# poja/Cattus

Measured on AMD Instinct MI355X. Metric: MCTS node-evals/sec (chess 20x256 net, batch 256), higher is better.
Workload: dtype f16x2

## Files before the change

cattus_amd/csrc/evaluator.hip:

```cpp
#include <hip/hip_runtime.h>

#include <algorithm>
#include <atomic>
#include <chrono>
#include <condition_variable>
#include <cmath>
#include <cstdarg>
#include <cstdio>
#include <cstdlib>
#include <cstring>
#include <deque>
#include <functional>
#include <map>
#include <memory>
#include <mutex>
#include <new>
#include <shared_mutex>
#include <string>
#include <thread>
#include <vector>

#include <dlfcn.h>

#include "../../include/cattus_hip.h"
// ... 49 lines not shown
    return f;
}

std::vector<int> choose_stream_shift(const cattus_net_desc& d, const float* p, int* t) {
    const uint32_t F = d.filters;
    const float* g0 = p + (size_t)F * d.planes * 9;
    const float* b0 = g0 + F;
    const size_t stem = (size_t)F * d.planes * 9 + 4 * F, block = (size_t)2 * F * F * 9 + 6 * F;
    std::vector<double> s(F);
    for (uint32_t c = 0; c < F; c++) s[c] = (double)g0[c] * g0[c] + (double)b0[c] * b0[c];
    for (uint32_t i = 0; i < d.blocks; i++) {
        const float* g2 = p + stem + i * block + (size_t)F * F * 9 + 2 * F + (size_t)F * F * 9;
        const float* b2 = g2 + F;
        for (uint32_t c = 0; c < F; c++) s[c] += (double)g2[c] * g2[c] + (double)b2[c] * b2[c];
    }
    *t = stream_shift_global(s);
    return stream_shifts(s);
}

void shift_folded(Folded& f, uint32_t cin, const std::vector<int>& tk, bool writes) {
    const size_t cout = f.b.size();
    for (size_t i = 0; i < f.w.size(); i++) f.w[i] = ldexpf(f.w[i], writes ? tk[i / cin % cout] : -tk[i % cin]);
    for (size_t co = 0; writes && co < cout; co++) f.b[co] = ldexpf(f.b[co], tk[co]);
}

struct DevArena {
    char* base = nullptr;
    size_t cap = 0, used = 0;
    ~DevArena() {
        if (base) (void)hipFree(base);
    }
    void* take(size_t bytes) {
        const size_t at = (used + 4095) & ~(size_t)4095;
        if (!base || at + bytes > cap) return nullptr;
        used = at + bytes;
        return base + at;
    }
};

struct DevBuf {
    void* p = nullptr;
    bool owned = true;
    ~DevBuf() {
        if (p && owned) (void)hipFree(p);
    }
    int alloc(size_t bytes, DevArena* arena = nullptr) {
        if (p && owned) (void)hipFree(p);
        p = nullptr, owned = true;
        if (arena && (p = arena->take(bytes ? bytes : 16))) {
            owned = false;
            return CATTUS_OK;
        }
        hipError_t e = hipMalloc(&p, bytes ? bytes : 16);
        if (e != hipSuccess) return fail(CATTUS_E_NOMEM, "hipMalloc(%zu) failed: %s", bytes, hipGetErrorString(e));
        return CATTUS_OK;
    }
    int upload(const void* src, size_t bytes, DevArena* arena = nullptr) {
        int rc = alloc(bytes, arena);
        if (rc) return rc;
        HIP_TRY(hipMemcpy(p, src, bytes, hipMemcpyHostToDevice));
        return CATTUS_OK;
    }
    template <typename T>
    T* as() const {
        return reinterpret_cast<T*>(p);
    }
};

struct PinnedBuf {
    void* p = nullptr;
    ~PinnedBuf() {
        if (p) (void)hipHostFree(p);
    }
    int alloc(size_t bytes) {
        hipError_t e = hipHostMalloc(&p, bytes ? bytes : 16, hipHostMallocDefault);
        if (e != hipSuccess) return fail(CATTUS_E_NOMEM, "hipHostMalloc(%zu) failed: %s", bytes, hipGetErrorString(e));
        return CATTUS_OK;
    }
    template <typename T>
    T* as() const {
        return reinterpret_cast<T*>(p);
    }
};

std::shared_mutex g_pin_mu;
std::map<const char*, size_t> g_pinned;
struct Roctx {
    int (*push)(const char*) = nullptr;
    int (*pop)() = nullptr;
    Roctx() {
        const char* on = getenv("CATTUS_ROCTX");
        if (!on || on[0] != '1') return;
        for (const char* name : {"librocprofiler-sdk-roctx.so", "libroctx64.so"}) {
            if (void* h = dlopen(name, RTLD_NOW | RTLD_GLOBAL)) {
                push = reinterpret_cast<int (*)(const char*)>(dlsym(h, "roctxRangePushA"));
                pop = reinterpret_cast<int (*)()>(dlsym(h, "roctxRangePop"));
                if (push && pop) return;
                push = nullptr, pop = nullptr;
            }
        }
    }
};
const Roctx& roctx() {
    static const Roctx r;
    return r;
}
struct RoctxRange {
    bool on;
    RoctxRange(const char* what, uint32_t n) : on(roctx().push != nullptr) {
        if (on) {
            char buf[64];
            snprintf(buf, sizeof buf, "%s n=%u", what, n);
            roctx().push(buf);
        }
    }
    ~RoctxRange() {
        if (on) roctx().pop();
    }
};

bool is_pinned(const void* p) {
    std::shared_lock<std::shared_mutex> lk(g_pin_mu);
    auto it = g_pinned.upper_bound((const char*)p);
    if (it == g_pinned.begin()) return false;
    --it;
    return (const char*)p < it->first + it->second;
}

struct ConvLayer { DevBuf w, b; };

struct ServerBatch {
    uint64_t seq = 0;
    uint32_t count = 0, collected = 0;
    bool sealed = false, running = false, done = false;
    int status = CATTUS_OK;
    std::string error;
    std::chrono::steady_clock::time_point t0;
    std::vector<uint64_t> planes;
    std::vector<float> policy, value;
    std::vector<uint8_t> taken;
};

constexpr int NLANES = CATTUS_HIP_LANES;

struct Lane {
    hipStream_t stream = nullptr;
    hipEvent_t done = nullptr;
    DevBuf d_planes, x0, a, t, y, hv, h1, d_policy, d_value;
    DevBuf d_legal_idx, d_legal_cnt, d_probs;
    uint32_t legal_stride = 0;
    PinnedBuf h_planes, h_policy, h_value;
    DevBuf tower_layers, tower_ready;
    PinnedBuf h_tower_err;
    std::mutex mu;
    ~Lane() {
        if (done) (void)hipEventDestroy(done);
        if (stream) (void)hipStreamDestroy(stream);
    }
};

enum class TowerKind {
    Simple,
    Generic,
    PerLayer,
    Resident64,
    Resident64Split,
    Wino16,
    Wino4,
};
struct TowerPlan {
    TowerKind kind = TowerKind::Generic;
    bool w_frag = false;
    bool inplace = false;
    bool one_launch = false;
    bool tuned() const { return kind != TowerKind::Simple && kind != TowerKind::Generic; }
    bool wino() const { return kind == TowerKind::Wino16 || kind == TowerKind::Wino4; }
};

}

struct cattus_eval {
    DevArena arena;
    cattus_net_desc d{};
    cattus_eval_config cfg{};
    TowerPlan plan;
    DevBuf d1w, d1b, d2w, d2b, svw, svb, spw, spb;
    bool wait_spin = true;
    Act act = Act::F32;
    uint32_t hw = 0, bpad = 0, cpad0 = 0;
    uint32_t slots = 64;
    uint32_t fpad = 0;
    DevBuf t64_layers, t64s_bias;
    bool t64s_fuse_heads = true;
    int t64s_depth = 0;
    bool pack_separately = false;
    int t64_force_ch = 0;
    std::atomic<bool> tower_gave_up{false};
    uint32_t persist_spin = 1u << 18, cus = 0;
    bool stream_shift_on = true;
    int stream_shift = 0;
    std::vector<int> stream_shifts;
    ConvOpts conv_opts;
    DevBuf d_saturated;
    bool t64_layer_steps = true;
    int device = 0;

    ConvLayer stem;
    std::vector<std::unique_ptr<ConvLayer>> c1, c2;
    DevBuf head_w, head_b, w1t, b1, w2, b2, wpt, bp;
    uint32_t kvp = 0, kpp = 0;

    Lane lanes[NLANES];
    std::atomic<unsigned> lane_rr{0};

    std::mutex stat_mu;
    cattus_stats stats{};
    uint64_t stats_tower_fallbacks = 0;

    std::mutex srv_mu;
    std::condition_variable srv_cv, done_cv;
    std::deque<std::unique_ptr<ServerBatch>> batches;
    uint64_t next_seq = 1;
    bool flush_req = false, stop = false;
    std::thread servers[NLANES];

    ~cattus_eval() {
        {
            std::lock_guard<std::mutex> lk(srv_mu);
            stop = true;
        }
        srv_cv.notify_all();
        done_cv.notify_all();
        for (auto& t : servers)
            if (t.joinable()) t.join();
    }
};

namespace {

size_t blob_floats(const cattus_net_desc& d) {
    const size_t hw = (size_t)d.board * d.board, F = d.filters;
    if (F == 0) {
        const size_t K = (size_t)d.planes * hw;
        return 2 * (K * K + K) + K + 1 + (size_t)d.moves * K + d.moves;
    }
    size_t n = F * d.planes * 9 + 4 * F;
    n += (size_t)d.blocks * (2 * F * F * 9 + 6 * F);
    n += (size_t)d.vhc * F + 2 * (size_t)d.vhc + (size_t)FC_HIDDEN * d.vhc * hw + FC_HIDDEN + FC_HIDDEN + 1;
    n += (size_t)d.phc * F + 2 * (size_t)d.phc + (size_t)d.moves * d.phc * hw + d.moves;
    return n;
}

std::mutex g_chain_mu;
hipEvent_t g_chain[64] = {};
int chain_persistent_launch(int device, hipStream_t st, const std::function<void()>& launch) {
    std::lock_guard<std::mutex> lk(g_chain_mu);
    hipEvent_t& ev = g_chain[device & 63];
    if (!ev) {
        HIP_TRY(hipEventCreateWithFlags(&ev, hipEventDisableTiming));
    } else {
        HIP_TRY(hipStreamWaitEvent(st, ev, 0));
    }
    launch();
    HIP_TRY(hipEventRecord(ev, st));
    return CATTUS_OK;
}

int upload_conv(cattus_eval* e, ConvLayer& L, const Folded& f, uint32_t cout, uint32_t cin, bool stem = false) {
    auto up = [](DevBuf& buf, const auto& v, DevArena* arena = nullptr) { return buf.upload(v.data(), v.size() * sizeof(v[0]), arena); };
    int rc;
    if (!e->plan.tuned()) return (rc = up(L.b, f.b)) ? rc : up(L.w, f.w);
    const ConvShape s{cout, cin, e->fpad, stem ? e->cpad0 : e->fpad};
    if (e->plan.wino() && !stem) {
        std::vector<int> sh;
        const std::vector<double> U = wino_transform(f, s, &sh);
        if ((rc = up(L.b, bias_and_scales(f, s, &sh)))) return rc;
        return up(L.w, wino_u(U, s, sh), &e->arena);
    }
    const bool scaled = act_f16_family(e->act);
    const std::vector<int> sh = scaled ? channel_shifts(f, s) : std::vector<int>();
    if ((rc = up(L.b, bias_and_scales(f, s, scaled ? &sh : nullptr)))) return rc;
    if (e->act == Act::F32) return up(L.w, rows_f32(f, s));
    if (e->act == Act::BF16) return up(L.w, rows_bf16(f, s));
    if (e->act == Act::F16) return up(L.w, rows_f16(f, s, sh));
    return e->plan.w_frag ? up(L.w, frag_f16x2(f, s, sh)) : up(L.w, rows_f16x2(f, s, sh));
}

int lane_common(cattus_eval* e, Lane& L) {
    const size_t B = e->cfg.max_batch, M = e->d.moves, plane_bytes = B * e->d.planes * e->cfg.plane_words * 8;
    int rc;
    HIP_TRY(hipStreamCreateWithFlags(&L.stream, hipStreamNonBlocking));
    HIP_TRY(hipEventCreateWithFlags(&L.done, hipEventBlockingSync | hipEventDisableTiming));
    if ((rc = L.d_planes.alloc(plane_bytes)) || (rc = L.d_policy.alloc(B * M * 4)) || (rc = L.d_value.alloc(B * 4))) return rc;
    if ((rc = L.h_planes.alloc(plane_bytes)) || (rc = L.h_policy.alloc(B * M * 4)) || (rc = L.h_value.alloc(B * 4))) return rc;
    return CATTUS_OK;
}

uint32_t hv_leaves(const cattus_eval* e) { return (e->bpad + 31) / 32 * 32; }

int build_simple(cattus_eval* e, const float* p) {
    const cattus_net_desc& d = e->d;
    const size_t K = (size_t)d.planes * e->hw, M = d.moves, B = e->cfg.max_batch;
    auto upload_t = [&](DevBuf& buf, const float* w, size_t n_out) -> int {
        std::vector<float> t(K * n_out);
        for (size_t n = 0; n < n_out; n++)
            for (size_t k = 0; k < K; k++) t[k * n_out + n] = w[n * K + k];
        return buf.upload(t.data(), t.size() * 4);
    };
    int rc;
    const float *w1 = p, *b1 = w1 + K * K, *w2 = b1 + K, *b2 = w2 + K * K, *vw = b2 + K, *vb = vw + K, *pw = vb + 1, *pb = pw + M * K;
    if ((rc = upload_t(e->d1w, w1, K)) || (rc = e->d1b.upload(b1, K * 4)) || (rc = upload_t(e->d2w, w2, K)) || (rc = e->d2b.upload(b2, K * 4)) ||
        (rc = upload_t(e->svw, vw, 1)) || (rc = e->svb.upload(vb, 4)) || (rc = upload_t(e->spw, pw, M)) || (rc = e->spb.upload(pb, M * 4)))
        return rc;
    for (Lane& L : e->lanes)
        if ((rc = lane_common(e, L)) || (rc = L.x0.alloc(B * K * 4)) || (rc = L.a.alloc(B * K * 4)) || (rc = L.t.alloc(B * K * 4))) return rc;
    return CATTUS_OK;
}

int build(cattus_eval* e, const float* p) {
    const cattus_net_desc& d = e->d;
    const TowerPlan& plan = e->plan;
    if (plan.kind == TowerKind::Simple) return build_simple(e, p);
    const uint32_t F = d.filters, hw = e->hw, FP = e->fpad;
    auto take = [&](size_t n) { return (p += n) - n; };
    int rc;
    e->stream_shifts.assign(F, 0);
    if (act_f16_family(e->act) && e->stream_shift_on) e->stream_shifts = choose_stream_shift(d, p, &e->stream_shift);
    const std::vector<int>& tk = e->stream_shifts;
    const bool shifted = std::any_of(tk.begin(), tk.end(), [](int t) { return t != 0; });
    {
        const float* w = take((size_t)F * d.planes * 9);
        const float *g = take(F), *be = take(F), *mu = take(F), *var = take(F);
        Folded f = fold_conv(w, F, d.planes, 9, g, be, mu, var);
        if (shifted) shift_folded(f, d.planes, tk, true);
        if ((rc = upload_conv(e, e->stem, f, F, d.planes, true))) return rc;
    }
    for (uint32_t i = 0; i < d.blocks; i++) {
        e->c1.emplace_back(new ConvLayer);
        e->c2.emplace_back(new ConvLayer);
        const float* w1 = take((size_t)F * F * 9);
        const float *mu1 = take(F), *var1 = take(F);
        Folded f1 = fold_conv(w1, F, F, 9, nullptr, nullptr, mu1, var1);
        if (shifted) shift_folded(f1, F, tk, false);
        if ((rc = upload_conv(e, *e->c1.back(), f1, F, F))) return rc;
        const float* w2 = take((size_t)F * F * 9);
        const float *g2 = take(F), *be2 = take(F), *mu2 = take(F), *var2 = take(F);
        Folded f2 = fold_conv(w2, F, F, 9, g2, be2, mu2, var2);
        if (shifted) shift_folded(f2, F, tk, true);
        if ((rc = upload_conv(e, *e->c2.back(), f2, F, F))) return rc;
    }
    std::vector<float> hw_w((size_t)(d.vhc + d.phc) * F), hw_b(std::max(32u, d.vhc + d.phc), 0.0f);
    const float* vw = take((size_t)d.vhc * F);
    const float *vmu = take(d.vhc), *vvar = take(d.vhc);
    Folded fv = fold_conv(vw, d.vhc, F, 1, nullptr, nullptr, vmu, vvar);
    const float* fc1_w = take((size_t)FC_HIDDEN * d.vhc * hw);
    const float* fc1_b = take(FC_HIDDEN);
    const float* fc2_w = take(FC_HIDDEN);
    const float* fc2_b = take(1);
    const float* pw = take((size_t)d.phc * F);
    const float *pmu = take(d.phc), *pvar = take(d.phc);
    Folded fp = fold_conv(pw, d.phc, F, 1, nullptr, nullptr, pmu, pvar);
    const float* pfc_w = take((size_t)d.moves * d.phc * hw);
    const float* pfc_b = take(d.moves);
    if (shifted) shift_folded(fv, F, tk, false), shift_folded(fp, F, tk, false);
    memcpy(hw_w.data(), fv.w.data(), fv.w.size() * 4);
    memcpy(hw_w.data() + fv.w.size(), fp.w.data(), fp.w.size() * 4);
    memcpy(hw_b.data(), fv.b.data(), fv.b.size() * 4);
    memcpy(hw_b.data() + fv.b.size(), fp.b.data(), fp.b.size() * 4);
    const uint32_t kv = d.vhc * hw, kp = d.phc * hw;
    if ((rc = e->head_b.upload(hw_b.data(), hw_b.size() * 4)) || (rc = e->b1.upload(fc1_b, FC_HIDDEN * 4)) || (rc = e->w2.upload(fc2_w, FC_HIDDEN * 4)) ||
        (rc = e->b2.upload(fc2_b, 4)) || (rc = e->bp.upload(pfc_b, d.moves * 4)))
        return rc;
    if (plan.tuned()) {
        const uint32_t ocn = d.vhc + d.phc;
        e->kvp = (kv + 15) / 16 * 16;
        e->kpp = (kp + 15) / 16 * 16;
        const uint32_t m32 = (d.moves + 31) / 32 * 32;
        std::vector<float> cw((size_t)32 * FP, 0.0f), w1((size_t)FC_HIDDEN * e->kvp, 0.0f), wp((size_t)m32 * e->kpp, 0.0f);
        for (uint32_t oc = 0; oc < ocn; oc++) memcpy(&cw[(size_t)oc * FP], &hw_w[(size_t)oc * F], (size_t)F * 4);
        for (uint32_t j = 0; j < FC_HIDDEN; j++) memcpy(&w1[(size_t)j * e->kvp], &fc1_w[(size_t)j * kv], kv * 4);
        for (uint32_t m = 0; m < d.moves; m++) memcpy(&wp[(size_t)m * e->kpp], &pfc_w[(size_t)m * kp], kp * 4);
        const Act hact = head_act(e->act);
        auto upload_t = [&](DevBuf& buf, const std::vector<float>& v) -> int {
            if (hact == Act::F32) return buf.upload(v.data(), v.size() * 4);
            std::vector<uint16_t> hb(v.size());
            for (size_t i = 0; i < v.size(); i++) hb[i] = f32_to_bf16(v[i]);
            return buf.upload(hb.data(), hb.size() * 2);
        };
        auto frag_order = [&](const std::vector<float>& v, uint32_t rows, uint32_t K) {
            const uint32_t kstep = hact == Act::F32 ? 8 : 16, half = kstep / 2;
            std::vector<float> o(v.size());
            for (uint32_t row = 0; row < rows; row++)
                for (uint32_t k = 0; k < K; k++)
                    o[((((size_t)(row >> 5) * (K / kstep) + k / kstep) * 2 + (k % kstep) / half) * 32 + (row & 31)) * half + k % half] =
                        v[(size_t)row * K + k];
            return o;
        };
        if ((rc = upload_t(e->head_w, cw)) || (rc = upload_t(e->w1t, frag_order(w1, FC_HIDDEN, e->kvp))) || (rc = upload_t(e->wpt, frag_order(wp, m32, e->kpp)))) return rc;
    } else {
        std::vector<float> w1t((size_t)kv * FC_HIDDEN), wpt((size_t)kp * d.moves);
        for (uint32_t j = 0; j < FC_HIDDEN; j++)
            for (uint32_t k = 0; k < kv; k++) w1t[(size_t)k * FC_HIDDEN + j] = fc1_w[(size_t)j * kv + k];
        for (uint32_t m = 0; m < d.moves; m++)
            for (uint32_t k = 0; k < kp; k++) wpt[(size_t)k * d.moves + m] = pfc_w[(size_t)m * kp + k];
        if ((rc = e->head_w.upload(hw_w.data(), hw_w.size() * 4)) || (rc = e->w1t.upload(w1t.data(), w1t.size() * 4)) || (rc = e->wpt.upload(wpt.data(), wpt.size() * 4))) return rc;
        e->kvp = kv, e->kpp = kp;
    }

    auto layer_table = [&](auto row) {
        std::vector<decltype(row(e->stem, 0, true))> tl{row(e->stem, 0, true)};
        for (uint32_t i = 0; i < d.blocks; i++) tl.push_back(row(*e->c1[i], 0, false)), tl.push_back(row(*e->c2[i], 1, false));
        return tl;
    };
    if (plan.kind == TowerKind::Resident64) {
        const auto tl = layer_table([](const ConvLayer& c, int res, bool) { return Tower64Layer{c.w.p, c.b.as<float>(), res, 0}; });
        if ((rc = e->t64_layers.upload(tl.data(), tl.size() * sizeof(Tower64Layer)))) return rc;
    }
    if (plan.kind == TowerKind::Resident64Split) {
        const auto tl = layer_table([](const ConvLayer& c, int res, bool stem) { return Tower64SplitLayer{c.w.p, c.b.as<float>(), res, stem ? 1 : 2}; });
        if ((rc = e->t64_layers.upload(tl.data(), tl.size() * sizeof(Tower64SplitLayer)))) return rc;
        if ((rc = e->t64s_bias.alloc(tl.size() * 512))) return rc;
        for (size_t l = 0; l < tl.size(); l++)
            HIP_TRY(hipMemcpy((char*)e->t64s_bias.p + l * 512, tl[l].bias, 512, hipMemcpyDeviceToDevice));
    }

    const bool tuned = plan.tuned();
    const size_t bpad = e->bpad, esz = tuned ? (act_f16_family(e->act) ? 4 : (size_t)act_bytes(e->act)) : 4;
    const size_t hesz = tuned ? (size_t)act_bytes(head_act(e->act)) : 4;
    const size_t slots = tuned ? e->slots : hw;
    for (Lane& L : e->lanes) {
        const size_t act_bytes_ = bpad * slots * FP * esz, hv_bytes = (size_t)(tuned ? hv_leaves(e) : bpad) * (e->kvp + e->kpp) * hesz;
        if ((rc = lane_common(e, L)) || (rc = L.x0.alloc(bpad * slots * e->cpad0 * esz)) || (rc = L.a.alloc(act_bytes_, &e->arena)) ||
            (rc = L.t.alloc(act_bytes_, &e->arena)) || (rc = L.y.alloc(act_bytes_, plan.inplace ? nullptr : &e->arena)) ||
            (rc = L.hv.alloc(hv_bytes)) || (rc = L.h1.alloc(bpad * FC_HIDDEN * 4)))
            return rc;
        HIP_TRY(hipMemset(L.hv.p, 0, hv_bytes));
        if (plan.one_launch) {
            std::vector<Wino4TowerLayer> tl;
            float *la = L.a.as<float>(), *lt = L.t.as<float>();
            for (uint32_t i = 0; i < d.blocks; i++) {
                tl.push_back(Wino4TowerLayer{la, e->c1[i]->w.p, e->c1[i]->b.as<float>(), nullptr, lt});
                tl.push_back(Wino4TowerLayer{lt, e->c2[i]->w.p, e->c2[i]->b.as<float>(), la, la});
            }
            if ((rc = L.tower_layers.upload(tl.data(), tl.size() * sizeof(Wino4TowerLayer))) || (rc = L.tower_ready.alloc(64 + (size_t)tl.size() * (bpad / 4) * 4)) ||
                (rc = L.h_tower_err.alloc(4)))
                return rc;
            *L.h_tower_err.as<unsigned>() = 0;
        }
    }
    return CATTUS_OK;
}

struct TowerTimer { std::vector<hipEvent_t> ev; size_t used = 0; };

bool one_launch_now(const cattus_eval* e, uint32_t nb) {
    return e->plan.one_launch && !e->tower_gave_up.load(std::memory_order_relaxed) && wino4_tower_fits(nb, e->fpad, e->cus);
}

struct Forward {
    cattus_eval* e;
    Lane& L;
    const uint64_t* d_planes;
    uint32_t n, nb;
    float *d_policy, *d_value;
    hipStream_t st;
    TowerTimer* tt;
    const cattus_net_desc& d = e->d;
    const uint32_t w64 = e->cfg.plane_words, S = d.board, F = d.filters, FP = e->fpad;
    float *a = L.a.as<float>(), *t = L.t.as<float>(), *y = L.y.as<float>();

    hipEvent_t ev() { return tt && tt->used < tt->ev.size() ? tt->ev[tt->used++] : nullptr; }

    void simple() {
        const uint32_t K = d.planes * e->hw;
        launch_planes_to_tensor_nchw(d_planes, n, d.planes, w64, S, n, L.x0.as<float>(), st);
        launch_dense(L.x0.as<float>(), K, e->d1w.as<float>(), e->d1b.as<float>(), n, K, K, a, 1, st);
        launch_dense(a, K, e->d2w.as<float>(), e->d2b.as<float>(), n, K, K, t, 1, st);
        launch_dense(t, K, e->svw.as<float>(), e->svb.as<float>(), n, K, 1, d_value, 2, st);
        launch_dense(t, K, e->spw.as<float>(), e->spb.as<float>(), n, K, d.moves, d_policy, 0, st);
    }

    const void* generic() {
        launch_planes_to_tensor_nchw(d_planes, n, d.planes, w64, S, n, L.x0.as<float>(), st);
        auto conv = [&](const ConvLayer& c, const float* in, uint32_t cin, const float* res, float* out) {
            hipEvent_t s0 = ev(), s1 = ev();
            launch_conv3x3_generic(in, c.w.as<float>(), c.b.as<float>(), res, out, n, cin, F, S, st, s0, s1);
        };
        conv(e->stem, L.x0.as<float>(), d.planes, nullptr, a);
        for (uint32_t i = 0; i < d.blocks; i++) {
            conv(*e->c1[i], a, F, nullptr, t);
            conv(*e->c2[i], t, F, a, y);
            std::swap(a, y);
        }
        return a;
    }

    template <class Args>
    void resident_args(Args& ta, bool fuse_heads) {
        ta.planes = d_planes, ta.layers = (decltype(ta.layers))e->t64_layers.p;
        ta.n = n, ta.C = d.planes, ta.w64 = w64, ta.S = S, ta.nlayers = 1 + 2 * d.blocks;
        if (!fuse_heads) return;
        ta.head_w = (decltype(ta.head_w))e->head_w.p, ta.hv = (decltype(ta.hv))L.hv.p;
        ta.head_b = e->head_b.as<float>();
        ta.hv_pol = hv_leaves(e) * e->kvp, ta.kvp = e->kvp, ta.kpp = e->kpp, ta.vhc = d.vhc, ta.ocn = d.vhc + d.phc;
    }

    void resident64() {
        Tower64Args ta{};
        resident_args(ta, true);
        const uint32_t rows = nb * e->slots;
        hipEvent_t s0 = ev(), s1 = ev();
        int ch = e->slots == 64 && rows / 64 <= 256 ? 4 : 2;
        if (e->t64_force_ch) ch = e->t64_force_ch == 4 && e->slots == 64 ? 4 : 2;
        launch_tower64(ta, rows, ch, e->t64_layer_steps, st, s0, s1);
    }

    const void* resident64_split() {
        Tower64SplitArgs ta{};
        resident_args(ta, e->t64s_fuse_heads);
        ta.sat = e->conv_opts.saturated, ta.bias_all = e->t64s_bias.as<float>();
        if (!e->t64s_fuse_heads) ta.out = a;
        hipEvent_t s0 = ev(), s1 = ev();
        launch_tower64_split(ta, nb * e->slots, e->t64s_depth, st, s0, s1);
        return ta.out;
    }

    void conv_mfma(const ConvLayer& c, const void* in, const void* res, void* out, int flags, bool stem = false) {
        const bool fused_stem = stem && stem_is_fused(d.planes, e->pack_separately);
        const StemInput stem_in{d_planes, n, d.planes, w64};
        if (stem && !fused_stem) launch_pack_planes_nhwc(e->act, d_planes, n, nb, d.planes, w64, S, e->cpad0, L.x0.p, st);
        hipEvent_t s0 = ev(), s1 = ev();
        launch_conv3x3_mfma(e->act, in, c.w.p, c.b.as<float>(), res, out, nb, stem ? e->cpad0 : FP, FP, S, st, s0, s1, fused_stem ? &stem_in : nullptr,
                            (e->plan.w_frag ? CONV_W_FRAG : 0) | flags, e->conv_opts);
    }

    const void* per_layer() {
        const int last_flags = act_f16_family(e->act) ? CONV_OUT_F32 : 0;
        conv_mfma(e->stem, L.x0.p, nullptr, a, d.blocks == 0 ? last_flags : 0, true);
        for (uint32_t i = 0; i < d.blocks; i++) {
            conv_mfma(*e->c1[i], a, nullptr, t, 0);
            conv_mfma(*e->c2[i], t, a, y, i + 1 == d.blocks ? last_flags : 0);
            std::swap(a, y);
        }
        return a;
    }

    int wino() {
        conv_mfma(e->stem, L.x0.p, nullptr, a, CONV_OUT_F32 | CONV_WINO_IN, true);
        if (one_launch_now(e, nb)) {
            hipEvent_t s0 = ev(), s1 = ev();
            unsigned* const tower_err = L.tower_ready.as<unsigned>();
            HIP_TRY(hipMemsetAsync(L.tower_ready.p, 0, 64 + (size_t)2 * d.blocks * (nb / 4) * 4, st));
            if (int crc = chain_persistent_launch(e->device, st, [&] {
                    launch_tower_wino4(L.tower_layers.as<Wino4TowerLayer>(), 2 * d.blocks, tower_err + 16, tower_err, e->conv_opts.saturated, nb, FP,
                                       e->persist_spin, e->cus, st, s0, s1);
                }))
                return crc;
            HIP_TRY(hipMemcpyAsync(L.h_tower_err.p, tower_err, 4, hipMemcpyDeviceToHost, st));
            return CATTUS_OK;
        }
        const auto launch = e->plan.kind == TowerKind::Wino4 ? launch_conv3x3_wino4 : launch_conv3x3_wino;
        auto conv = [&](const ConvLayer& c, const float* in, const float* res, float* out) {
            hipEvent_t s0 = ev(), s1 = ev();
            launch(in, c.w.p, c.b.as<float>(), res, out, nb, FP, FP, st, s0, s1, e->conv_opts.saturated);
        };
        for (uint32_t i = 0; i < d.blocks; i++) {
            conv(*e->c1[i], a, nullptr, t);
            conv(*e->c2[i], t, a, e->plan.inplace ? a : y);
            if (!e->plan.inplace) std::swap(a, y);
        }
        return CATTUS_OK;
    }

    void heads_mfma(const void* tower) {
        HeadsMfma hd{};
        hd.conv_w = e->head_w.p, hd.conv_b = e->head_b.as<float>(), hd.hv = L.hv.p;
        hd.w1 = e->w1t.p, hd.b1 = e->b1.as<float>(), hd.h1 = L.h1.as<float>();
        hd.wp = e->wpt.p, hd.bp = e->bp.as<float>(), hd.policy = d_policy;
        hd.hw = e->hw, hd.vhc = d.vhc, hd.phc = d.phc, hd.kvp = e->kvp, hd.kpp = e->kpp, hd.M = d.moves;
        hd.w2 = e->w2.as<float>(), hd.b2 = e->b2.as<float>(), hd.value = d_value;
        hd.slots = e->slots, hd.hv_leaves = hv_leaves(e);
        launch_heads_mfma(head_act(e->act), tower, n, FP, hd, st);
    }

    void heads_generic(const void* tower) {
        const uint32_t hw = e->hw, kv = d.vhc * hw, kp = d.phc * hw;
        TowerView tv;
        tv.x = tower, tv.act = Act::F32, tv.sb = F * hw, tv.sk = hw, tv.sp = 1;
        launch_head_conv1x1(tv, e->head_w.as<float>(), e->head_b.as<float>(), n, F, d.vhc + d.phc, hw, L.hv.as<float>(), st);
        launch_value_fc1(L.hv.as<float>(), kv + kp, e->w1t.as<float>(), e->b1.as<float>(), n, kv, L.h1.as<float>(), st);
        launch_value_fc2_tanh(L.h1.as<float>(), e->w2.as<float>(), e->b2.as<float>(), n, d_value, st);
        launch_policy_fc(L.hv.as<float>(), kv + kp, kv, e->wpt.as<float>(), e->bp.as<float>(), n, kp, d.moves, d_policy, st);
    }
};

int enqueue_forward(cattus_eval* e, Lane& L, const uint64_t* d_planes, uint32_t n, float* d_policy, float* d_value, hipStream_t st, TowerTimer* tt = nullptr) {
    const uint32_t bpw = e->plan.tuned() ? ROWS_PER_WG / e->slots : 1;
    Forward f{e, L, d_planes, n, (n + bpw - 1) / bpw * bpw, d_policy, d_value, st, tt};
    switch (e->plan.kind) {
        case TowerKind::Simple: f.simple(); break;
        case TowerKind::Generic: f.heads_generic(f.generic()); break;
        case TowerKind::PerLayer: f.heads_mfma(f.per_layer()); break;
        case TowerKind::Resident64: f.resident64(), f.heads_mfma(nullptr); break;
        case TowerKind::Resident64Split: f.heads_mfma(f.resident64_split()); break;
        case TowerKind::Wino16:
        case TowerKind::Wino4:
            if (int rc = f.wino()) return rc;
            f.heads_mfma(f.a);
            break;
    }
    if (hipError_t err = hipGetLastError()) return fail(CATTUS_E_DEVICE, "kernel launch failed: %s", hipGetErrorString(err));
    return CATTUS_OK;
}

void account(cattus_eval* e, uint32_t n, const double* seconds) {
    std::lock_guard<std::mutex> lk(e->stat_mu);
    cattus_stats& s = e->stats;
    if (seconds) {
        s.run_seconds_ema = 0.01 * s.run_seconds_ema + 0.99 * *seconds;
        s.run_seconds_total += *seconds;
    }
    s.batches += 1;
    s.positions += n;
    if (n == e->cfg.max_batch) s.full_batches += 1;
}

bool take_tower_give_up(cattus_eval* e, Lane& L) {
    if (!L.h_tower_err.p || *L.h_tower_err.as<volatile unsigned>() == 0) return false;
    *L.h_tower_err.as<volatile unsigned>() = 0;
    e->tower_gave_up.store(true, std::memory_order_relaxed);
    std::lock_guard<std::mutex> sl(e->stat_mu);
    e->stats_tower_fallbacks += 1;
    return true;
}

struct LegalArgs {
    const uint16_t* idx;
    const uint16_t* cnt;
    uint32_t stride;
    float* probs;
};

int eval_host(cattus_eval* e, const uint64_t* planes, uint32_t n, float* policy, float* value, const LegalArgs* lg = nullptr) {
    const cattus_net_desc& d = e->d;
    std::unique_lock<std::mutex> lk;
    Lane* lane = nullptr;
    for (Lane& cand : e->lanes) {
        std::unique_lock<std::mutex> tl(cand.mu, std::try_to_lock);
        if (tl.owns_lock()) {
            lane = &cand, lk = std::move(tl);
            break;
        }
    }
    if (!lane) {
        lane = &e->lanes[e->lane_rr.fetch_add(1) % NLANES];
        lk = std::unique_lock<std::mutex>(lane->mu);
    }
    Lane& L = *lane;
    const RoctxRange range(lg ? "cattus_hip_eval_legal" : "cattus_hip_eval", n);
    HIP_TRY(hipSetDevice(e->device));
    const auto t0 = std::chrono::steady_clock::now();
    const size_t pbytes = (size_t)n * d.planes * e->cfg.plane_words * 8;
    const bool direct = is_pinned(planes) && (lg || is_pinned(policy)) && is_pinned(value);
    if (lg && (L.legal_stride < lg->stride || !L.d_probs.p)) {
        const size_t B = e->cfg.max_batch;
        int arc;
        if ((arc = L.d_legal_idx.alloc(B * lg->stride * 2)) || (arc = L.d_legal_cnt.alloc(B * 2)) ||
            (arc = L.d_probs.alloc(B * lg->stride * 4)))
            return arc;
        L.legal_stride = lg->stride;
    }
    const void* src_planes = planes;
    if (!direct) {
        memcpy(L.h_planes.p, planes, pbytes);
        src_planes = L.h_planes.p;
    }
    HIP_TRY(hipMemcpyAsync(L.d_planes.p, src_planes, pbytes, hipMemcpyHostToDevice, L.stream));
    auto copy_out = [&]() -> int {
        if (lg) {
            HIP_TRY(hipMemcpyAsync(L.d_legal_idx.p, lg->idx, (size_t)n * lg->stride * 2, hipMemcpyHostToDevice, L.stream));
            HIP_TRY(hipMemcpyAsync(L.d_legal_cnt.p, lg->cnt, (size_t)n * 2, hipMemcpyHostToDevice, L.stream));
            if (launch_legal_softmax(L.d_policy.as<float>(), d.moves, L.d_legal_idx.as<uint16_t>(), L.d_legal_cnt.as<uint16_t>(),
                                     lg->stride, n, L.d_probs.as<float>(), L.stream))
                return fail(CATTUS_E_INVALID, "legal stride %u exceeds 1024", lg->stride);
            HIP_TRY(hipMemcpyAsync(lg->probs, L.d_probs.p, (size_t)n * lg->stride * 4, hipMemcpyDeviceToHost, L.stream));
        } else {
            HIP_TRY(hipMemcpyAsync(direct ? (void*)policy : L.h_policy.p, L.d_policy.p, (size_t)n * d.moves * 4, hipMemcpyDeviceToHost, L.stream));
        }
        HIP_TRY(hipMemcpyAsync(direct ? (void*)value : L.h_value.p, L.d_value.p, (size_t)n * 4, hipMemcpyDeviceToHost, L.stream));
        return CATTUS_OK;
    };
    auto run_batch = [&]() -> int {
        int rc = enqueue_forward(e, L, L.d_planes.as<uint64_t>(), n, L.d_policy.as<float>(), L.d_value.as<float>(), L.stream);
        if (rc) return rc;
        if ((rc = copy_out())) return rc;
        if (e->wait_spin) {
            HIP_TRY(hipStreamSynchronize(L.stream));
        } else {
            HIP_TRY(hipEventRecord(L.done, L.stream));
            HIP_TRY(hipEventSynchronize(L.done));
        }
        return CATTUS_OK;
    };
    int rc = run_batch();
    if (rc) return rc;
    if (take_tower_give_up(e, L) && (rc = run_batch())) return rc;
    if (!direct) {
        if (!lg) memcpy(policy, L.h_policy.p, (size_t)n * d.moves * 4);
        memcpy(value, L.h_value.p, (size_t)n * 4);
    }
    const double seconds = std::chrono::duration<double>(std::chrono::steady_clock::now() - t0).count();
// ... 558 lines not shown
```

cattus_amd/csrc/kernels.h:

```cpp
#pragma once
#include <hip/hip_runtime.h>
#include <stdint.h>

#include "frag_index.h"

namespace cattus {

inline uint32_t tower_slots(uint32_t S) { return S <= 8 ? 64u : 128u; }
constexpr int ROWS_PER_WG = 256;
constexpr int COUT_PER_WG = 64;

enum class Act : int { F32 = 0, BF16 = 1, F16S = 2, F16 = 3 };

inline bool act_two_bytes(Act a) { return a == Act::BF16 || a == Act::F16; }
inline int act_bytes(Act a) { return act_two_bytes(a) ? 2 : 4; }
inline int act_kc(Act a) { return act_two_bytes(a) ? 64 : 32; }
inline Act head_act(Act a) { return a == Act::BF16 ? Act::BF16 : Act::F32; }
inline bool act_f16_family(Act a) { return a == Act::F16S || a == Act::F16; }

hipError_t prepare_device();

void launch_pack_planes_nhwc(Act act, const uint64_t* planes, uint32_t n, uint32_t bpad, uint32_t C,
                             uint32_t w64, uint32_t S, uint32_t cpad, void* out, hipStream_t st);
void launch_planes_to_tensor_nchw(const uint64_t* planes, uint32_t n, uint32_t C, uint32_t w64, uint32_t S,
                                  uint32_t batch, float* out, hipStream_t st);

struct StemInput {
    const uint64_t* planes;
    uint32_t n, C, w64;
};
constexpr int CONV_OUT_F32 = 1, CONV_W_FRAG = 2, CONV_WINO_IN = 4;
constexpr float WINO_ACT_MAX = 16376.0f;
struct ConvOpts {
    int cb = 0;
    int pbw = 0;
    unsigned* saturated = nullptr;
};
void launch_conv3x3_mfma(Act act, const void* in, const void* w, const float* bias, const void* res, void* out,
                         uint32_t bpad, uint32_t cin, uint32_t cout, uint32_t S, hipStream_t st,
                         hipEvent_t ev_start = nullptr, hipEvent_t ev_stop = nullptr, const StemInput* stem = nullptr,
                         int flags = 0, const ConvOpts& opts = ConvOpts());

bool wino_supported(uint32_t bpad, uint32_t cin, uint32_t cout, uint32_t S);
void launch_conv3x3_wino(const float* in, const void* wu, const float* bias, const float* res, float* out, uint32_t bpad, uint32_t cin,
                         uint32_t cout, hipStream_t st, hipEvent_t ev_start, hipEvent_t ev_stop, unsigned* sat);
hipError_t prepare_wino();

bool wino4_supported(uint32_t bpad, uint32_t cin, uint32_t cout, uint32_t S);
void launch_conv3x3_wino4(const float* in, const void* wu, const float* bias, const float* res, float* out, uint32_t bpad, uint32_t cin,
                          uint32_t cout, hipStream_t st, hipEvent_t ev_start, hipEvent_t ev_stop, unsigned* sat);
hipError_t prepare_wino4();
struct Wino4TowerLayer {
    const float* in;
    const void* wu;
    const float* bias;
    const float* res;
    float* out;
};
bool wino4_tower_fits(uint32_t bpad, uint32_t filters, uint32_t cus);
void launch_tower_wino4(const Wino4TowerLayer* d_layers, uint32_t nlayers, unsigned* ready, unsigned* err, unsigned* sat, uint32_t bpad, uint32_t filters,
                        uint32_t spin_budget, uint32_t cus, hipStream_t st, hipEvent_t ev_start, hipEvent_t ev_stop);

double launch_mfma_sustain(Act act, int cus, int iters, float* out, hipStream_t st);

struct Tower64Layer {
    const void* w;
    const float* bias;
    int res;
    int pad_;
};
struct Tower64Args {
    const uint64_t* planes;
    const Tower64Layer* layers;
    void* out;
    uint32_t n, C, w64, S, nlayers;
    const void* head_w;
    const float* head_b;
    void* hv;
    uint32_t hv_pol, kvp, kpp, vhc, ocn;
};
void launch_tower64(const Tower64Args& args, uint32_t rows, int ch, bool layer_steps, hipStream_t st,
                    hipEvent_t ev_start = nullptr, hipEvent_t ev_stop = nullptr);

struct Tower64SplitLayer {
    const void* wf;
    const float* bias;
    int res;
    int nch;
};
struct Tower64SplitArgs {
    const uint64_t* planes;
    const Tower64SplitLayer* layers;
    const float* bias_all;
    float* out;
    unsigned* sat;
    uint32_t n, C, w64, S, nlayers;
    const float* head_w;
    const float* head_b;
    float* hv;
    uint32_t hv_pol, kvp, kpp, vhc, ocn;
};
constexpr int T64S_MAX_LAYERS = 81;
void launch_tower64_split(const Tower64SplitArgs& args, uint32_t rows, int shape, hipStream_t st, hipEvent_t ev_start = nullptr,
                          hipEvent_t ev_stop = nullptr);
hipError_t prepare_tower64_split();

void launch_conv3x3_generic(const float* in, const float* w, const float* bias, const float* res, float* out,
                            uint32_t b, uint32_t cin, uint32_t cout, uint32_t S, hipStream_t st,
                            hipEvent_t ev_start = nullptr, hipEvent_t ev_stop = nullptr);

struct HeadsMfma {
    const void* conv_w;
    const float* conv_b;
    void* hv;
    const void* w1;
    const float* b1;
    float* h1;
    const void* wp;
    const float* bp;
    float* policy;
    const float *w2, *b2;
    float* value;
    uint32_t hw, vhc, phc, kvp, kpp, M;
    uint32_t hv_leaves;
    uint32_t slots;
};
void launch_heads_mfma(Act act, const void* tower, uint32_t nb, uint32_t F, const HeadsMfma& hd, hipStream_t st);

struct TowerView {
    const void* x;
    Act act;
    uint32_t sb, sk, sp;
};
void launch_head_conv1x1(TowerView x, const float* w, const float* bias, uint32_t b, uint32_t F, uint32_t ocn,
                         uint32_t hw, float* hv, hipStream_t st);
void launch_value_fc1(const float* hv, uint32_t hv_stride, const float* w1t, const float* b1, uint32_t b, uint32_t K,
                      float* h1, hipStream_t st);
void launch_value_fc2_tanh(const float* h1, const float* w2, const float* b2, uint32_t b, float* value,
                           hipStream_t st);
int launch_legal_softmax(const float* policy, uint32_t M, const uint16_t* idx, const uint16_t* cnt, uint32_t L, uint32_t b,
                         float* probs, hipStream_t st);
void launch_policy_fc(const float* hv, uint32_t hv_stride, uint32_t off, const float* wpt, const float* bp, uint32_t b,
                      uint32_t K, uint32_t M, float* policy, hipStream_t st);
void launch_dense(const float* x, uint32_t x_stride, const float* wt, const float* bias, uint32_t b, uint32_t K, uint32_t N,
                  float* y, int epi, hipStream_t st);

}
```

cattus_amd/csrc/kernels_wino4.hip:

```cpp
#include "kernels.h"
#include "device_common.h"

#include <hip/hip_ext.h>

namespace cattus {

constexpr int W4_TROW = 8 * SP;
constexpr int W4_IMG = 9472;
constexpr int W4_ZAREA = 512;
constexpr int W4_IMGZ = W4_IMG + W4_ZAREA;
constexpr int W4_DBUF = 8 * W4_IMGZ;
constexpr int W4_LDS_LOOP = 2 * W4_DBUF;
constexpr int W4_LDS_Z = 4 * 2 * 64 * 256;
constexpr int W4_LDS_TOTAL = W4_LDS_Z > W4_LDS_LOOP ? W4_LDS_Z : W4_LDS_LOOP;
static_assert(W4_IMG % 256 == 0 && W4_IMGZ % 256 == 0 && W4_DBUF % 256 == 0, "the zero area keeps a read's banks only if everything is 256-B aligned");
static_assert(W4_IMG >= 8 * W4_TROW + 16 && W4_ZAREA >= 256 + 128 && W4_LDS_LOOP <= 160 * 1024, "image / zero area / LDS sizes");

typedef __attribute__((ext_vector_type(2))) _Float16 w4_f16x2;

template <int V>
using w4_int = std::integral_constant<int, V>;

#ifdef CATTUS_STAMPS
__device__ unsigned long long g_stamps_w4[1024 * 4 * 10];
// ... 235 lines not shown
                    asm volatile("s_waitcnt vmcnt(8)"
                                 : "+v"(r0), "+v"(r1), "+v"(r2), "+v"(r3), "+v"(pend[0]), "+v"(pend[1]), "+v"(pend[2]), "+v"(pend[3]), "+v"(pend[4]),
                                   "+v"(pend[5]), "+v"(pend[6]), "+v"(pend[7]));
                } else asm volatile("s_waitcnt vmcnt(8)" : "+v"(r0), "+v"(r1), "+v"(r2), "+v"(r3));
                ring[l][0] = r0, ring[l][1] = r1, ring[l][2] = r2, ring[l][3] = r3;
            }
            const frag uh0 = __builtin_bit_cast(frag, ring[l][0]), ul0 = __builtin_bit_cast(frag, ring[l][1]);
            const frag uh1 = __builtin_bit_cast(frag, ring[l][2]), ul1 = __builtin_bit_cast(frag, ring[l][3]);
            const frag vh = __builtin_bit_cast(frag, l < 2 ? vh01[tbv][l] : vh23[SP_][tbv][l - 2]);
            const frag vl = __builtin_bit_cast(frag, l < 2 ? vl01[tbv][l] : vl23[SP_][tbv][l - 2]);
            const int gp = 6 * i + 36;
            auto gap = [&](int e) __attribute__((always_inline)) {
                const int ph = (gp + e) / 24, j = (gp + e) % 24;
                __builtin_amdgcn_sched_barrier(0);
                slot(ph == 1 ? SP_ : SP_ ^ 1, ph == 2 ? 0 : 1, j);
                if (SP_ == 0 && i >= 4 && 6 * (i - 4) + e < 16) t_unit(pend, wdst + (uint32_t)(bufstep > 0 ? W4_DBUF : 0), 6 * (i - 4) + e);
                const int le = (i & 1) ? e : e - 2;
                if (le >= 0 && le < 4) {
                    if (i == 0) load_u1(ring[3][le], wcur, 3, le);
                    if (i == 3 && !LAST) load_u1(ring[0][le], wnext, 0, le);
                    if (i == 4 && !LAST) load_u1(ring[1][le], wnext, 1, le);
                    if (i == 7 && !LAST) load_u1(ring[2][le], wnext, 2, le);
                }
                if (SP_ == 1 && !LAST) {
                    if (i == 5) load_piece(pend[e], ch_next, e);
                    if (i == 6 && (e == 2 || e == 3)) load_piece(pend[4 + e], ch_next, 4 + e);
                }
                __builtin_amdgcn_sched_barrier(0);
            };
            Mfma<T>::mac(ul0, vh, acc[l][tbv][0]);
            gap(0);
            Mfma<T>::mac(ul1, vh, acc[l][tbv][1]);
            gap(1);
            Mfma<T>::mac(uh0, vl, acc[l][tbv][0]);
            gap(2);
            Mfma<T>::mac(uh1, vl, acc[l][tbv][1]);
            gap(3);
            Mfma<T>::mac(uh0, vh, acc[l][tbv][0]);
            gap(4);
            Mfma<T>::mac(uh1, vh, acc[l][tbv][1]);
            gap(5);
        }
    };
    W4_STAMP(1);
    int c = 0;
    do {
        const char* w1 = wks + (size_t)16 * SW_STAGE;
        const char* w2 = wks + (size_t)(c + 1 < nch ? 32 : 16) * SW_STAGE;
        kstep(wks, w1, 0, w4_int<0>{}, w4_int<0>{});
        kstep(w1, w2, min(c + 2, nch - 1), w4_int<1>{}, w4_int<0>{});
        wks = w2;
    } while (++c < nch);
    W4_STAMP(2);
    __builtin_amdgcn_sched_barrier(0);

    int elane = lane;
    asm volatile("" : "+v"(elane));
    const int en = elane & 31, eh = elane >> 5;
    const int board = elane >> 4, pc = elane & 15;
    typedef const __attribute__((address_space(1))) f32x4 w4_gf32x4;
    const f32x4 bias4 = *(w4_gf32x4*)(bias + cout0 + pc * 4);
    const f32x4 ds4 = *(w4_gf32x4*)(bias + cout + cout0 + pc * 4);
    const size_t orow = (size_t)row0 + board * 64 + q * 16;
    const uint32_t cstride = (uint32_t)cout * 4;
    const uint32_t evoff = (uint32_t)((board * 64 + q * 16) * cout + pc * 4) * 4;
    const char* rbase = reinterpret_cast<const char*>(res + (size_t)row0 * cout + cout0);
    char* obase = reinterpret_cast<char*>(out + (size_t)row0 * cout + cout0);
    f32x4 skip[16];
    auto load_skip = [&](int k) __attribute__((always_inline)) {
        if (PERSIST) asm volatile("global_load_dwordx4 %0, %1, %2 sc1" : "=&v"(skip[k]) : "v"(evoff + k * cstride), "s"(rbase) : "memory");
        else skip[k] = *reinterpret_cast<const f32x4*>(res + (orow + k) * (size_t)cout + cout0 + pc * 4);
    };
    W4_STAMP(3);
    asm volatile("s_barrier" ::: "memory");
#pragma unroll
    for (int tbv = 0; tbv < 2; tbv++)
#pragma unroll
        for (int cb = 0; cb < 2; cb++)
#pragma unroll
            for (int g = 0; g < 4; g++) {
                if (has_res) load_skip(tbv * 8 + cb * 4 + g);
                f32x4 m[4];
#pragma unroll
                for (int l = 0; l < 4; l++)
#pragma unroll
                    for (int e = 0; e < 4; e++) asm volatile("v_accvgpr_read_b32 %0, %1" : "=v"(m[l][e]) : "a"(acc[l][tbv][cb][g * 4 + e]));
                const f32x4 z0 = m[0] + m[1] + m[2], z1 = m[1] - m[2] - m[3];
                const int unit = (cb * 8 + g * 2 + eh) ^ (en & 15);
                char* zp = smem + ((size_t)(q * 2) * 64 + tbv * 32 + en) * 256 + (unit << 4);
                *reinterpret_cast<f32x4*>(zp) = z0;
                *reinterpret_cast<f32x4*>(zp + 64 * 256) = z1;
            }
    asm volatile("s_waitcnt vmcnt(0)"
                 : "+v"(ring[0][0]), "+v"(ring[0][1]), "+v"(ring[0][2]), "+v"(ring[0][3]), "+v"(ring[1][0]), "+v"(ring[1][1]), "+v"(ring[1][2]),
                   "+v"(ring[1][3]), "+v"(ring[2][0]), "+v"(ring[2][1]), "+v"(ring[2][2]), "+v"(ring[2][3]), "+v"(ring[3][0]), "+v"(ring[3][1]),
                   "+v"(ring[3][2]), "+v"(ring[3][3]), "+v"(pend[0]), "+v"(pend[1]), "+v"(pend[2]), "+v"(pend[3]), "+v"(pend[4]), "+v"(pend[5]),
                   "+v"(pend[6]), "+v"(pend[7])::"memory");
    if (PERSIST && has_res) {
        asm volatile(""
                     : "+v"(skip[0]), "+v"(skip[1]), "+v"(skip[2]), "+v"(skip[3]), "+v"(skip[4]), "+v"(skip[5]), "+v"(skip[6]), "+v"(skip[7]), "+v"(skip[8]),
                       "+v"(skip[9]), "+v"(skip[10]), "+v"(skip[11]), "+v"(skip[12]), "+v"(skip[13]), "+v"(skip[14]), "+v"(skip[15]));
    }
    asm volatile("s_waitcnt lgkmcnt(0)\n\ts_barrier" ::: "memory");
    W4_STAMP(4);
#pragma unroll
    for (int k = 0; k < 16; k++) {
        const int rp = k >> 3, txo = (k & 7) >> 1, cp = k & 1;
        const int tile16 = q * 4 + txo;
        const char* zb = smem + ((size_t)cp * 64 + board * 16 + tile16) * 256 + ((pc ^ tile16) << 4);
        const f32x4 za = *reinterpret_cast<const f32x4*>(zb + (size_t)(rp + 0) * 2 * 64 * 256);
        const f32x4 zc = *reinterpret_cast<const f32x4*>(zb + (size_t)(rp + 1) * 2 * 64 * 256);
        const f32x4 zd = *reinterpret_cast<const f32x4*>(zb + (size_t)(rp + 2) * 2 * 64 * 256);
        const f32x4 a = rp == 0 ? za + zc + zd : za - zc - zd;
        f32x4 v;
#pragma unroll
        for (int j = 0; j < 4; j++) {
            float x = __builtin_fmaf(a[j], ds4[j], bias4[j]);
            if (has_res) x = x + skip[k][j];
            x = x > 0.0f ? x : 0.0f;
            v[j] = x < WINO_ACT_MAX ? x : WINO_ACT_MAX;
        }
        vmax = fmaxf(fmaxf(vmax, fmaxf(v[0], v[1])), fmaxf(v[2], v[3]));
        if (PERSIST) asm volatile("global_store_dwordx4 %0, %1, %2 sc1\n\ts_nop 1" ::"v"(evoff + k * cstride), "v"(v), "s"(obase) : "memory");
        else *reinterpret_cast<f32x4*>(out + (orow + k) * (size_t)cout + cout0 + pc * 4) = v;
    }
    if (vmax >= WINO_ACT_MAX) atomicAdd(sat, 1u);
    if (PERSIST) {
        asm volatile("s_waitcnt vmcnt(0)" ::: "memory");
        W4_STAMP(9);
        asm volatile("s_barrier" ::: "memory");
        if (tid == 0) __hip_atomic_fetch_add(sync.done_word, 1u, __ATOMIC_RELAXED, __HIP_MEMORY_SCOPE_AGENT);
    }
#ifdef CATTUS_STAMPS
    W4_STAMP(5);
    W4_STAMP_RT(7);
    if (lane == 0 && blockIdx.x < 1024) {
#pragma unroll
        for (int i = 0; i < 10; i++) g_stamps_w4[((size_t)blockIdx.x * 4 + q) * 10 + i] = st_[i];
    }
#endif
}

template <bool HAS_RES>
__global__ void __launch_bounds__(256, 1)
    conv3x3_wino4_kernel(const float* __restrict__ in, const _Float16* __restrict__ wu, const float* __restrict__ bias,
                         const float* res, float* out, unsigned* __restrict__ sat, int cin, int cout) {
    extern __shared__ __attribute__((aligned(16))) char smem[];
    const W4Sync none{};
    w4_layer<HAS_RES ? 1 : 0, false>(in, wu, bias, res, out, sat, cin, cout, smem, none, (int)blockIdx.x, (int)gridDim.x);
}

__global__ void __launch_bounds__(256, 1)
    tower_wino4_kernel(const Wino4TowerLayer* __restrict__ layers, int nlayers, unsigned* ready, unsigned* err, unsigned* __restrict__ sat, int filters,
                       unsigned spin_budget, int tiles) {
    extern __shared__ __attribute__((aligned(16))) char smem[];
    const int ncg = filters >> 6, ngroups = tiles / ncg;
    auto group_of = [&](int wg) {
        int logical = wg;
        if ((tiles & 7) == 0) logical = (wg & 7) * (tiles >> 3) + (wg >> 3);
        return logical / ncg;
    };
    auto sync_of = [&](int layer, int group) {
        W4Sync sync;
        sync.wait_word = layer > 0 ? ready + (size_t)(layer - 1) * ngroups + group : nullptr;
        sync.done_word = ready + (size_t)layer * ngroups + group;
        sync.err = err, sync.wait_target = (unsigned)ncg, sync.spin_budget = spin_budget;
        return sync;
    };
    for (int layer = 0; layer + 1 < nlayers; layer += 2) {
        const Wino4TowerLayer A = layers[layer];
        for (int wg = blockIdx.x; wg < tiles; wg += gridDim.x)
            w4_layer<0, true>(A.in, reinterpret_cast<const _Float16*>(A.wu), A.bias, nullptr, A.out, sat, filters, filters, smem, sync_of(layer, group_of(wg)), wg, tiles);
        const Wino4TowerLayer B = layers[layer + 1];
        for (int wg = blockIdx.x; wg < tiles; wg += gridDim.x)
            w4_layer<1, true>(B.in, reinterpret_cast<const _Float16*>(B.wu), B.bias, B.res, B.out, sat, filters, filters, smem, sync_of(layer + 1, group_of(wg)), wg, tiles);
    }
}

bool wino4_supported(uint32_t bpad, uint32_t cin, uint32_t cout, uint32_t S) {
    return S == 8 && cin >= 128 && cin % 32 == 0 && cout >= 128 && cout % 64 == 0 && bpad % 4 == 0;
}

template <class F>
static void for_each_wino4(F&& f) {
    each_bool([&](auto r) { f(&conv3x3_wino4_kernel<decltype(r)::value>, r); });
}

void launch_conv3x3_wino4(const float* in, const void* wu, const float* bias, const float* res, float* out, uint32_t bpad, uint32_t cin,
                          uint32_t cout, hipStream_t st, hipEvent_t ev_start, hipEvent_t ev_stop, unsigned* sat) {
    typedef _Float16 H;
    const dim3 grid((bpad / 4) * (cout / 64));
    for_each_wino4([&](auto kernel, auto r) {
        if (r == (res != nullptr))
            hipExtLaunchKernelGGL(kernel, grid, dim3(256), W4_LDS_TOTAL, st, ev_start, ev_stop, 0, in, (const H*)wu, bias, res, out, sat, (int)cin, (int)cout);
    });
}

static uint32_t tower_grid(uint32_t tiles, uint32_t cus) { return tiles <= cus ? tiles : cus & ~7u; }

bool wino4_tower_fits(uint32_t bpad, uint32_t filters, uint32_t cus) {
    const uint32_t tiles = (bpad / 4) * (filters / 64);
    return tiles <= cus || (cus >= 8 && tiles % 8 == 0);
}

void launch_tower_wino4(const Wino4TowerLayer* d_layers, uint32_t nlayers, unsigned* ready, unsigned* err, unsigned* sat, uint32_t bpad, uint32_t filters,
                        uint32_t spin_budget, uint32_t cus, hipStream_t st, hipEvent_t ev_start, hipEvent_t ev_stop) {
    const uint32_t tiles = (bpad / 4) * (filters / 64);
    hipExtLaunchKernelGGL(tower_wino4_kernel, dim3(tower_grid(tiles, cus)), dim3(256), W4_LDS_TOTAL, st, ev_start, ev_stop, 0, d_layers, (int)nlayers, ready, err,
                          sat, (int)filters, spin_budget, (int)tiles);
}

#ifdef CATTUS_STAMPS
extern "C" __attribute__((visibility("default"))) int cattus_hip_debug_stamps_w4(unsigned long long* out, size_t n) {
    return (int)hipMemcpyFromSymbol(out, HIP_SYMBOL(g_stamps_w4), n * sizeof(unsigned long long));
}
#endif

hipError_t prepare_wino4() {
    hipError_t err = hipSuccess;
    for_each_wino4([&](auto kernel, auto) { lds_opt_in(err, kernel, W4_LDS_TOTAL); });
    lds_opt_in(err, &tower_wino4_kernel, W4_LDS_TOTAL);
    return err;
}

}
```

Before: 216,100.

## Double-buffer tower ready flags, clear in-kernel, and report errors via mapped host word

Removes the per-launch hipMemsetAsync of the persistent tower's ready flags by alternating between two banks. Each launch zeroes the other bank inside the kernel prologue. It also drops the per-launch D2H memcpy of the error word: the kernel writes a system-scope store to the mapped pinned host word when an error occurred. The chain event wait is skipped when the same stream launches consecutively. Together these cut two stream operations and one cross-stream wait per forward pass. The cost is reliance on correct bank alternation and on mapped host memory being visible to the device.

```diff
diff --git a/cattus_amd/csrc/evaluator.hip b/cattus_amd/csrc/evaluator.hip
--- a/cattus_amd/csrc/evaluator.hip
+++ b/cattus_amd/csrc/evaluator.hip
@@ -225,6 +225,7 @@
     PinnedBuf h_planes, h_policy, h_value;
     DevBuf tower_layers, tower_ready;
     PinnedBuf h_tower_err;
+    uint32_t tower_bank_words = 0, tower_launches = 0;
     std::mutex mu;
     ~Lane() {
         if (done) (void)hipEventDestroy(done);
@@ -326,16 +327,19 @@
 
 std::mutex g_chain_mu;
 hipEvent_t g_chain[64] = {};
+hipStream_t g_chain_stream[64] = {};
 int chain_persistent_launch(int device, hipStream_t st, const std::function<void()>& launch) {
     std::lock_guard<std::mutex> lk(g_chain_mu);
     hipEvent_t& ev = g_chain[device & 63];
+    hipStream_t& last = g_chain_stream[device & 63];
     if (!ev) {
         HIP_TRY(hipEventCreateWithFlags(&ev, hipEventDisableTiming));
-    } else {
+    } else if (st != last || st == hipStreamPerThread) {
         HIP_TRY(hipStreamWaitEvent(st, ev, 0));
     }
     launch();
     HIP_TRY(hipEventRecord(ev, st));
+    last = st;
     return CATTUS_OK;
 }
 
@@ -515,10 +519,15 @@
                 tl.push_back(Wino4TowerLayer{la, e->c1[i]->w.p, e->c1[i]->b.as<float>(), nullptr, lt});
                 tl.push_back(Wino4TowerLayer{lt, e->c2[i]->w.p, e->c2[i]->b.as<float>(), la, la});
             }
-            if ((rc = L.tower_layers.upload(tl.data(), tl.size() * sizeof(Wino4TowerLayer))) || (rc = L.tower_ready.alloc(64 + (size_t)tl.size() * (bpad / 4) * 4)) ||
-                (rc = L.h_tower_err.alloc(4)))
+            L.tower_bank_words = (uint32_t)(tl.size() * (bpad / 4));
+            const size_t ready_bytes = 64 + (size_t)2 * L.tower_bank_words * 4;
+            if ((rc = L.tower_layers.upload(tl.data(), tl.size() * sizeof(Wino4TowerLayer))) || (rc = L.tower_ready.alloc(ready_bytes)) || (rc = L.h_tower_err.alloc(4)))
                 return rc;
+            HIP_TRY(hipMemset(L.tower_ready.p, 0, ready_bytes));
             *L.h_tower_err.as<unsigned>() = 0;
+            void* host_word = nullptr;
+            HIP_TRY(hipHostGetDevicePointer(&host_word, L.h_tower_err.p, 0));
+            HIP_TRY(hipMemcpy(L.tower_ready.as<unsigned>() + WINO4_ERR_HOST_WORD, &host_word, sizeof host_word, hipMemcpyHostToDevice));
         }
     }
     return CATTUS_OK;
@@ -623,13 +632,14 @@
         if (one_launch_now(e, nb)) {
             hipEvent_t s0 = ev(), s1 = ev();
             unsigned* const tower_err = L.tower_ready.as<unsigned>();
-            HIP_TRY(hipMemsetAsync(L.tower_ready.p, 0, 64 + (size_t)2 * d.blocks * (nb / 4) * 4, st));
+            unsigned* const bank = tower_err + 16 + (size_t)(L.tower_launches & 1) * L.tower_bank_words;
+            unsigned* const other = tower_err + 16 + (size_t)(~L.tower_launches & 1) * L.tower_bank_words;
             if (int crc = chain_persistent_launch(e->device, st, [&] {
-                    launch_tower_wino4(L.tower_layers.as<Wino4TowerLayer>(), 2 * d.blocks, tower_err + 16, tower_err, e->conv_opts.saturated, nb, FP,
-                                       e->persist_spin, e->cus, st, s0, s1);
+                    launch_tower_wino4(L.tower_layers.as<Wino4TowerLayer>(), 2 * d.blocks, bank, other, L.tower_bank_words, tower_err,
+                                       e->conv_opts.saturated, nb, FP, e->persist_spin, e->cus, st, s0, s1);
                 }))
                 return crc;
-            HIP_TRY(hipMemcpyAsync(L.h_tower_err.p, tower_err, 4, hipMemcpyDeviceToHost, st));
+            L.tower_launches += 1;
             return CATTUS_OK;
         }
         const auto launch = e->plan.kind == TowerKind::Wino4 ? launch_conv3x3_wino4 : launch_conv3x3_wino;
diff --git a/cattus_amd/csrc/kernels.h b/cattus_amd/csrc/kernels.h
--- a/cattus_amd/csrc/kernels.h
+++ b/cattus_amd/csrc/kernels.h
@@ -58,8 +58,10 @@
     float* out;
 };
 bool wino4_tower_fits(uint32_t bpad, uint32_t filters, uint32_t cus);
-void launch_tower_wino4(const Wino4TowerLayer* d_layers, uint32_t nlayers, unsigned* ready, unsigned* err, unsigned* sat, uint32_t bpad, uint32_t filters,
-                        uint32_t spin_budget, uint32_t cus, hipStream_t st, hipEvent_t ev_start, hipEvent_t ev_stop);
+constexpr int WINO4_ERR_HOST_WORD = 2;
+void launch_tower_wino4(const Wino4TowerLayer* d_layers, uint32_t nlayers, unsigned* ready, unsigned* ready_next, uint32_t next_words, unsigned* err,
+                        unsigned* sat, uint32_t bpad, uint32_t filters, uint32_t spin_budget, uint32_t cus, hipStream_t st, hipEvent_t ev_start,
+                        hipEvent_t ev_stop);
 
 double launch_mfma_sustain(Act act, int cus, int iters, float* out, hipStream_t st);
 
diff --git a/cattus_amd/csrc/kernels_wino4.hip b/cattus_amd/csrc/kernels_wino4.hip
--- a/cattus_amd/csrc/kernels_wino4.hip
+++ b/cattus_amd/csrc/kernels_wino4.hip
@@ -411,8 +411,9 @@
 
 __global__ void __launch_bounds__(256, 1)
     tower_wino4_kernel(const Wino4TowerLayer* __restrict__ layers, int nlayers, unsigned* ready, unsigned* err, unsigned* __restrict__ sat, int filters,
-                       unsigned spin_budget, int tiles) {
+                       unsigned spin_budget, int tiles, unsigned* ready_next, unsigned next_words) {
     extern __shared__ __attribute__((aligned(16))) char smem[];
+    for (unsigned i = blockIdx.x * 256 + threadIdx.x; i < next_words; i += gridDim.x * 256) ready_next[i] = 0;
     const int ncg = filters >> 6, ngroups = tiles / ncg;
     auto group_of = [&](int wg) {
         int logical = wg;
@@ -433,6 +434,11 @@
         const Wino4TowerLayer B = layers[layer + 1];
         for (int wg = blockIdx.x; wg < tiles; wg += gridDim.x)
             w4_layer<1, true>(B.in, reinterpret_cast<const _Float16*>(B.wu), B.bias, B.res, B.out, sat, filters, filters, smem, sync_of(layer + 1, group_of(wg)), wg, tiles);
+    }
+    if (threadIdx.x == 0) {
+        unsigned bad;
+        asm volatile("global_load_dword %0, %1, off sc1\n\ts_waitcnt vmcnt(0)" : "=v"(bad) : "v"(err) : "memory");
+        if (bad != 0) __hip_atomic_store(*reinterpret_cast<unsigned**>(err + WINO4_ERR_HOST_WORD), 1u, __ATOMIC_RELAXED, __HIP_MEMORY_SCOPE_SYSTEM);
     }
 }
 
@@ -462,11 +468,12 @@
     return tiles <= cus || (cus >= 8 && tiles % 8 == 0);
 }
 
-void launch_tower_wino4(const Wino4TowerLayer* d_layers, uint32_t nlayers, unsigned* ready, unsigned* err, unsigned* sat, uint32_t bpad, uint32_t filters,
-                        uint32_t spin_budget, uint32_t cus, hipStream_t st, hipEvent_t ev_start, hipEvent_t ev_stop) {
+void launch_tower_wino4(const Wino4TowerLayer* d_layers, uint32_t nlayers, unsigned* ready, unsigned* ready_next, uint32_t next_words, unsigned* err,
+                        unsigned* sat, uint32_t bpad, uint32_t filters, uint32_t spin_budget, uint32_t cus, hipStream_t st, hipEvent_t ev_start,
+                        hipEvent_t ev_stop) {
     const uint32_t tiles = (bpad / 4) * (filters / 64);
     hipExtLaunchKernelGGL(tower_wino4_kernel, dim3(tower_grid(tiles, cus)), dim3(256), W4_LDS_TOTAL, st, ev_start, ev_stop, 0, d_layers, (int)nlayers, ready, err,
-                          sat, (int)filters, spin_budget, (int)tiles);
+                          sat, (int)filters, spin_budget, (int)tiles, ready_next, next_words);
 }
 
 #ifdef CATTUS_STAMPS
```

After: 217,400 (median of 6 runs). About the same (+0.6%).
